# uniio/ivf-hnsw

Hardware: AMD Instinct MI355X
Metric: queries/sec @ Recall@1, SIFT1B PQ16 nprobe=32; ADC scan HBM GB/s vs peak (higher is better)
Workload: dtype f32

## Files before the change

### ivf-hnsw_amd/csrc/capi_internal.h

```cpp
#pragma once
#include "../../include/ivfhnsw_hip.h"
#include "ivfhnsw_kernels.h"

#include <hip/hip_runtime.h>

#include <algorithm>
#include <new>
#include <cmath>
#include <cstddef>
#include <cstdio>
#include <cstdlib>
#include <cstring>
#include <functional>
#include <string>
#include <unordered_map>
#include <vector>

namespace ivfhnsw_gpu_impl {

int fail(int code, const char *fmt, ...) __attribute__((format(printf, 2, 3)));

#define HIP_TRY(expr)                                                                                        \
    do {                                                                                                     \
        hipError_t e_ = (expr);                                                                              \
// ... 359 lines not shown
        if (!on)
            return;
        (void)hipEventRecord(ev.b, s);
        h->pending.push_back(ev);
    }
};

constexpr uint32_t kHeapStreamCap = 8192;

constexpr int kSplitAuto = 1000;

constexpr size_t kMaxBatchAll = 1 << 17;

struct EarlyTables {
    hipStream_t stream;
    hipEvent_t ready;
    hipEvent_t done;
};

struct SearchCall {
    uint32_t *status_out = nullptr;
    bool defer_redo = false;
    bool no_latency = false;
    bool wrote_status = false;
    const EarlyTables *early = nullptr;
};

struct WalkClear {
    uint64_t *keys = nullptr;
    uint32_t *done = nullptr;
    bool cleared = false;
};

struct SearchArgs {
    size_t nq, k;
    const float *d_queries;
    const uint32_t *d_coarse_ids;
    const float *d_coarse_dists;
    const ivfhnsw_search_params *p;
    float *d_distances;
    int64_t *d_labels, *d_out_keys;
    const uint8_t *d_query_slots = nullptr;
    SearchArgs slice(size_t q0, size_t n, size_t d) const
    {
        return {n, k, d_queries + q0 * d, d_coarse_ids ? d_coarse_ids + q0 * p->nprobe : nullptr,
                d_coarse_dists ? d_coarse_dists + q0 * p->nprobe : nullptr, p, d_distances + q0 * k, d_labels + q0 * k,
                d_out_keys, d_query_slots ? d_query_slots + q0 : nullptr};
    }
};

struct Chunk : SearchArgs {
    int nprobe, max_seg, plan_k;
    bool heap_big;
    ScanFilter fmask;
    const float *xq;
    const uint32_t *cid;
    const float *cd;
    bool use_tail;
    WalkClear meet;
    int nsplit;
    bool heap, pipe;
    const EarlyTables *early;
};

int search_args_guard(const ivfhnsw_gpu *h, const ivfhnsw_search_params *p, size_t k);
int stage_in(ivfhnsw_gpu *h, DevBuf &b, const void *src, size_t bytes);
int stage_out(ivfhnsw_gpu *h, void *dst, const DevBuf &b, size_t bytes);
int chunk_checks(ivfhnsw_gpu *h, const Chunk &c, bool results = true);
int chunk_workspace(ivfhnsw_gpu *h, Chunk &c);
int chunk_coarse(ivfhnsw_gpu *h, Chunk &c, const SearchCall &call);
int chunk_plan_table(ivfhnsw_gpu *h, Chunk &c);

void base_filter_drop(ivfhnsw_gpu *h);
int base_filter_cols(ivfhnsw_gpu *h, const ivfhnsw_gpu *b, SweepCols *cols, size_t *nx);

void base_slots_drop(ivfhnsw_gpu *h);
int base_slots_table_write(ivfhnsw_gpu *h, bool create);
int base_slots_call(ivfhnsw_gpu *h, const ivfhnsw_gpu *b, const char *who, const StripCols **table, unsigned *forms);

void range_drop(ivfhnsw_gpu *h);

int grouping_dedupe_reserve(ivfhnsw_gpu *h);
int grouping_dedupe_dev(ivfhnsw_gpu *h, const uint32_t *d_sizes, const uint32_t *d_nn, int *dedupe);

int encode_rows(ivfhnsw_gpu *h, size_t m, float *dx, const float *table, const uint32_t *rows);
int encode_groups_impl(ivfhnsw_gpu *h, size_t ngroups, size_t nsubc, const uint32_t *centroid_idx,
                       const uint64_t *offsets, const float *x, size_t efSearch, uint32_t *out_nn_centroid_idxs,
                       float *out_alphas, uint32_t *out_subcentroid_idxs, uint8_t *out_codes, uint8_t *out_norm_codes,
                       bool dev, bool stage);

}
```

### ivf-hnsw_amd/csrc/capi_search.cpp

```cpp
#include "capi_internal.h"

static size_t env_size(const char *name, size_t def)
{
    const char *e = getenv(name);
    return (e && *e) ? (size_t)atol(e) : def;
}

int ivfhnsw_gpu_impl::search_args_guard(const ivfhnsw_gpu *h, const ivfhnsw_search_params *p, size_t k)
{
    if (!h->has_ivf)
        return fail(IVFHNSW_ERR_STATE, "search before upload_ivf");
    if (!p || p->nprobe == 0 || k == 0)
        return fail(IVFHNSW_ERR_INVALID, "nprobe and k must be positive");
    return IVFHNSW_OK;
}

int ivfhnsw_gpu_impl::stage_in(ivfhnsw_gpu *h, DevBuf &b, const void *src, size_t bytes)
{
    int rc = b.ensure(bytes);
    if (rc)
        return rc;
    HIP_TRY(hipMemcpyAsync(b.p, src, bytes, hipMemcpyHostToDevice, h->stream));
    return IVFHNSW_OK;
}

int ivfhnsw_gpu_impl::stage_out(ivfhnsw_gpu *h, void *dst, const DevBuf &b, size_t bytes)
{
    HIP_TRY(hipMemcpyAsync(dst, b.p, bytes, hipMemcpyDeviceToHost, h->stream));
    return IVFHNSW_OK;
}

static int walk_scratch(ivfhnsw_gpu *h, size_t words, size_t nslots, size_t nq, uint32_t **tails)
{
    int rc = h->w_visited.ensure(words * sizeof(uint32_t) * std::max<size_t>(nslots, 64) * 2);
    if (rc)
        return rc;
    if (h->w_visited.p != h->walk.zero_ptr || h->w_visited.bytes != h->walk.zero_bytes) {
        HIP_TRY(hipMemsetAsync(h->w_visited.p, 0, h->w_visited.bytes, h->stream));
        h->walk.zero = true;
        h->walk.zero_ptr = h->w_visited.p;
        h->walk.zero_bytes = h->w_visited.bytes;
    }
    *tails = reinterpret_cast<uint32_t *>(h->w_visited.as<char>() + h->w_visited.bytes / 2);
    return h->w_redo.ensure(nq * sizeof(uint32_t));
}

static int coarse_dev_impl(ivfhnsw_gpu *h, size_t nq, const float *d_queries, size_t nprobe, size_t efSearch,
                           uint32_t *d_coarse_ids, float *d_coarse_dists, const SearchCall &call, WalkClear &meet)
{
    int rc = bind(h);
    if (rc)
        return rc;
    if (!h->has_graph)
        return fail(IVFHNSW_ERR_STATE, "coarse search needs upload_quantizer");
    if (nprobe == 0 || efSearch < nprobe)
        return fail(IVFHNSW_ERR_INVALID, "efSearch %zu < nprobe %zu (precondition of IndexIVF_HNSW.cpp:249-258)",
                    efSearch, nprobe);
    if (efSearch > 1024)
        return fail(IVFHNSW_ERR_INVALID, "efSearch %zu > 1024 unsupported on the device", efSearch);
    if (nq == 0)
        return IVFHNSW_OK;
    if (nq > 0x7fffffffull)
        return fail(IVFHNSW_ERR_INVALID, "nq too large");
    const size_t words = ((((size_t)h->gr.n + 31) / 32) + 3) & ~(size_t)3;
    StageScope sc(h, IVFHNSW_STAGE_COARSE);
    static const size_t lat_max_nq = env_size("IVFHNSW_LATENCY_MAX_NQ", 256);
    StatusWords *st = status_words(h);
    uint32_t *tails = nullptr;
    if (!call.no_latency && nq <= lat_max_nq && coarse_latency_supported(h->gr, (int)efSearch)) {
        uint32_t *hdr = &st->redo_len;
        const bool defer = call.defer_redo;
        if (!defer) {
            if ((rc = walk_scratch(h, words, 64, nq, &tails)))
                return rc;
            HIP_TRY(hipMemsetAsync(hdr, 0, 3 * sizeof(uint32_t), h->stream));
        }
        HIP_TRY(launch_coarse_latency(h->stream, h->gr, d_queries, (int)nq, (int)nprobe, (int)efSearch, d_coarse_ids,
                                      d_coarse_dists, status_word(h), meet.keys, meet.done, defer ? nullptr : hdr,
                                      defer ? nullptr : h->w_redo.as<uint32_t>()));
        meet.cleared = meet.keys != nullptr;
        if (!defer)
            HIP_TRY(launch_coarse_redo(h->stream, h->gr, d_queries, (int)nq, (int)nprobe, (int)efSearch, d_coarse_ids,
                                       d_coarse_dists, h->w_visited.as<uint32_t>(), words, status_word(h), hdr,
                                       h->w_redo.as<uint32_t>(), tails, 64));
        return IVFHNSW_OK;
    }
    const int nslots = (int)std::min<size_t>(nq, (size_t)coarse_slots_for((int)efSearch));
    if ((rc = walk_scratch(h, words, (size_t)nslots, nq, &tails)))
        return rc;
    HIP_TRY(launch_coarse(h->stream, h->gr, d_queries, (int)nq, (int)nprobe, (int)efSearch, d_coarse_ids, d_coarse_dists,
                          h->w_visited.as<uint32_t>(), words, nslots, status_word(h), &st->walk_next,
                          h->w_visited.bytes / 2, &h->walk.zero, h->w_redo.as<uint32_t>(), tails, 64,
                          &h->walk.counters_clean));
    return IVFHNSW_OK;
}

int ivfhnsw_gpu_coarse_dev(ivfhnsw_gpu *h, size_t nq, const float *d_queries, size_t nprobe, size_t efSearch,
                           uint32_t *d_coarse_ids, float *d_coarse_dists)
{
    WalkClear meet;
    return coarse_dev_impl(h, nq, d_queries, nprobe, efSearch, d_coarse_ids, d_coarse_dists, SearchCall(), meet);
}

int ivfhnsw_gpu_rotate_dev(ivfhnsw_gpu *h, size_t nq, const float *d_queries, float *d_out)
{
    int rc = bind(h);
    if (rc)
        return rc;
    if (!h->has_ivf)
        return fail(IVFHNSW_ERR_STATE, "rotate needs upload_ivf");
    if (nq == 0)
        return IVFHNSW_OK;
    if (!d_queries || !d_out || nq > 0x7fffffffull)
        return fail(IVFHNSW_ERR_INVALID, "null buffer or nq too large");
    if (h->t.opq_At) {
        StageScope sc(h, IVFHNSW_STAGE_OPQ);
        HIP_TRY(launch_opq(h->stream, h->t.opq_At, d_queries, d_out, (int)nq, h->t.d));
    } else if (d_out != d_queries) {
        HIP_TRY(hipMemcpyAsync(d_out, d_queries, nq * (size_t)h->t.d * sizeof(float), hipMemcpyDeviceToDevice, h->stream));
    }
    return IVFHNSW_OK;
}

int ivfhnsw_gpu_coarse(ivfhnsw_gpu *h, size_t nq, const float *queries, size_t k, size_t efSearch, uint32_t *ids,
                       float *dists)
{
// ... 225 lines not shown
    return IVFHNSW_OK;
}

int ivfhnsw_gpu_impl::chunk_coarse(ivfhnsw_gpu *h, Chunk &c, const SearchCall &call)
{
    const size_t nq = c.nq;
    int rc;
    c.xq = c.d_queries;
    if (h->t.opq_At) {
        if ((rc = h->w_xq.ensure(nq * (size_t)h->t.d * sizeof(float))))
            return rc;
        {
            StageScope sc(h, IVFHNSW_STAGE_OPQ);
            HIP_TRY(launch_opq(h->stream, h->t.opq_At, c.d_queries, h->w_xq.as<float>(), (int)nq, h->t.d));
        }
        c.xq = h->w_xq.as<float>();
        if (call.early) {
            HIP_TRY(hipEventRecord(call.early->ready, h->stream));
            HIP_TRY(hipStreamWaitEvent(call.early->stream, call.early->ready, 0));
        }
    }
    static const size_t tail_max_nq = env_size("IVFHNSW_TAIL_MAX_NQ", 8);
    c.use_tail = !h->has_group && nq <= tail_max_nq && !c.d_out_keys && !c.fmask.any() &&
                 ivf_tail_supported(h->t, c.nprobe, (int)c.k);
    if (c.use_tail) {
        if ((rc = h->w_tail.ensure(nq * (sizeof(uint64_t) + sizeof(uint32_t)))))
            return rc;
        c.meet.keys = h->w_tail.as<uint64_t>();
        c.meet.done = reinterpret_cast<uint32_t *>(c.meet.keys + nq);
    }
    c.cid = c.d_coarse_ids;
    c.cd = c.d_coarse_dists;
    if (!c.cid) {
        if ((rc = h->w_cid.ensure(nq * (size_t)c.nprobe * sizeof(uint32_t))) ||
            (rc = h->w_cd.ensure(nq * (size_t)c.nprobe * sizeof(float))) ||
            (rc = coarse_dev_impl(h, nq, c.xq, c.p->nprobe, c.p->efSearch, h->w_cid.as<uint32_t>(), h->w_cd.as<float>(),
                                  call, c.meet)))
            return rc;
        c.cid = h->w_cid.as<uint32_t>();
        c.cd = h->w_cd.as<float>();
    }
    return IVFHNSW_OK;
}

static int chunk_tail(ivfhnsw_gpu *h, const Chunk &c, SearchCall &call)
{
    const size_t nq = c.nq;
    const int nsplit = (int)std::min<size_t>(32, (2048 + nq - 1) / nq);
    StageScope sc(h, IVFHNSW_STAGE_SCAN);
    if (!c.meet.cleared)
        HIP_TRY(hipMemsetAsync(c.meet.keys, 0, nq * (sizeof(uint64_t) + sizeof(uint32_t)), h->stream));
    HIP_TRY(launch_ivf_tail(h->stream, h->t, c.xq, c.cid, c.cd, (int)nq, c.nprobe, c.p->max_codes, nsplit, c.meet.keys,
                            c.meet.done, h->w_hdr.as<PlanHdr>(), c.d_distances, c.d_labels, status_word(h),
                            call.status_out));
    call.wrote_status = call.status_out != nullptr;
    remember_plan(h, nq, c.max_seg, false, "ivf_tail_kernel");
    return IVFHNSW_OK;
}

int ivfhnsw_gpu_impl::chunk_plan_table(ivfhnsw_gpu *h, Chunk &c)
{
    const int nq = (int)c.nq, max_seg = c.max_seg;
    const ivfhnsw_search_params *p = c.p;
    int rc;
    c.heap = p->heap_order && c.k > 1;
    c.nsplit = (c.k == 1 && c.nq < 1024) ? (int)std::min<size_t>(32, (2048 + c.nq - 1) / c.nq) : 1;
    c.pipe = c.k == 1 && !h->has_group && !c.heap && !c.fmask.any() && h->opt_scan_pipe != 0 &&
             scan_pipe_supported(h->t, max_seg, nq, c.nsplit, h->n_local > 0, h->opt_scan_pipe == 1);
    const bool plan_lut = !c.pipe && plan_lut_shape(h);
    if (!c.pipe && (rc = h->w_luts.ensure(c.nq * (size_t)h->t.M * 256 * sizeof(float))))
        return rc;
    const PlanView plan = plan_of(h, max_seg, c.nq);
    uint64_t *keys = h->w_keys.as<uint64_t>();
    if (plan_lut && c.early) {
        const EarlyTables &e = *c.early;
        {
            StageScope sc(h, IVFHNSW_STAGE_LUT, e.stream);
            HIP_TRY(launch_lut(e.stream, h->t, c.xq, h->w_luts.as<float>(), nq, nullptr));
        }
        HIP_TRY(hipEventRecord(e.done, e.stream));
        {
            StageScope sc(h, IVFHNSW_STAGE_PLAN);
            HIP_TRY(launch_plan_ivf(h->stream, h->t, c.cid, c.cd, c.nprobe, p->max_codes, plan, keys, c.plan_k));
        }
        HIP_TRY(hipStreamWaitEvent(h->stream, e.done, 0));
        return IVFHNSW_OK;
    }
    if (plan_lut) {
        StageScope sc(h, IVFHNSW_STAGE_LUT);
        HIP_TRY(launch_plan_lut(h->stream, h->t, c.xq, c.cid, c.cd, c.nprobe, p->max_codes, plan, keys, c.plan_k,
                                h->w_luts.as<float>()));
        return IVFHNSW_OK;
    }
    {
        StageScope sc(h, IVFHNSW_STAGE_PLAN);
        if (h->has_group) {
            if ((rc = h->w_qsd.ensure(c.nq * (size_t)max_seg * 2 * sizeof(float))))
                return rc;
            HIP_TRY(launch_plan_grouping(h->stream, h->t, h->g, h->gr, c.xq, c.cid, c.cd, c.nprobe, p->max_codes,
                                         p->do_pruning, plan, keys, c.plan_k, h->w_qsd.as<float>()));
        } else {
            HIP_TRY(launch_plan_ivf(h->stream, h->t, c.cid, c.cd, c.nprobe, p->max_codes, plan, keys, c.plan_k));
        }
    }
    if (!c.pipe) {
        StageScope sc(h, IVFHNSW_STAGE_LUT);
        HIP_TRY(launch_lut(h->stream, h->t, c.xq, h->w_luts.as<float>(), nq, plan.hdr));
    }
    return IVFHNSW_OK;
}

static int chunk_scan_select(ivfhnsw_gpu *h, const Chunk &c)
{
    const int k = (int)c.k;
    const bool heap = c.heap, replay_here = c.heap && !c.d_out_keys;
    float *luts = h->w_luts.as<float>();
    const PlanView plan = plan_of(h, c.max_seg, c.nq);
    int rc;
    float *heap_ws = nullptr;
    if (replay_here) {
        if ((rc = h->w_heap.ensure(heap_scan_ws_bytes(h->t.M, k, plan.nq))))
            return rc;
        heap_ws = h->w_heap.as<float>();
    }
    if (c.heap_big) {
        {
            StageScope sc(h, IVFHNSW_STAGE_SCAN);
            HIP_TRY(launch_heap_scan(h->stream, h->t, luts, plan, k, nullptr, nullptr, heap_ws, c.d_distances, c.d_labels,
                                     c.fmask));
        }
        remember_plan(h, c.nq, c.max_seg, false, c.fmask.name("heap_scan_kernel", "heap_scan_kernel+filter", "heap_scan_kernel+slots"));
        return IVFHNSW_OK;
    }
    if (heap) {
        if ((rc = h->w_stream.ensure(c.nq * (size_t)kHeapStreamCap * sizeof(uint64_t))) ||
// ... 263 lines not shown
```

### ivf-hnsw_amd/csrc/ivfhnsw_kernels.h

```cpp
#pragma once

#include <hip/hip_runtime.h>
#include <mutex>
#include <stdint.h>

#include "scan_dispatch.h"
#include "sweep_plan_math.h"
#include "update_math.h"

namespace ivfhnsw_gpu_impl {

struct DynLdsState {
    std::mutex m;
    size_t raised[64] = {};
};
inline hipError_t raise_dyn_lds(const void *kern, size_t bytes, DynLdsState &st)
{
    int dev = 0;
    hipError_t e = hipGetDevice(&dev);
    if (e != hipSuccess)
        return e;
    if (dev < 0 || dev >= 64)
        return hipFuncSetAttribute(kern, hipFuncAttributeMaxDynamicSharedMemorySize, (int)bytes);
    std::lock_guard<std::mutex> lk(st.m);
// ... 123 lines not shown
                       const char **kernel_name);
bool scan_pipe_supported(const IvfTables &t, int max_seg, int nq, int nsplit, bool has_codes, bool forced = false);
hipError_t launch_scan_pipe(hipStream_t s, const IvfTables &t, const float *xq, const PlanView &p, uint64_t *keys);
bool ivf_tail_supported(const IvfTables &t, int nprobe, int k);
hipError_t launch_ivf_tail(hipStream_t s, const IvfTables &t, const float *xq, const uint32_t *cid, const float *cd,
                           int nq, int nprobe, uint64_t max_codes, int nsplit, uint64_t *keys_inv, uint32_t *done,
                           PlanHdr *hdr, float *dist, int64_t *labels, const uint32_t *status_word, uint32_t *status_out);
hipError_t launch_heap_replay(hipStream_t s, const IvfTables &t, const PlanView &p, const uint64_t *stream,
                              const uint32_t *stream_len, uint32_t stream_cap, int k, float *dist, int64_t *labels,
                              uint32_t *status,
                              int64_t *out_keys = nullptr,
                              uint32_t *redo_hdr = nullptr, uint32_t *redo_list = nullptr);
bool heap_scan_lds_tier(int code_size, int k);
size_t heap_scan_ws_bytes(int code_size, int k, int nq);
hipError_t launch_heap_scan(hipStream_t s, const IvfTables &t, const float *luts, const PlanView &p, int k,
                            uint32_t *redo_hdr, const uint32_t *redo_list, float *heap_ws, float *dist, int64_t *labels,
                            const ScanFilter &fmask = ScanFilter());
hipError_t launch_range_count(hipStream_t s, const IvfTables &t, const float *luts, const PlanView &p, int nsplit,
                              int seg_len_hint, float radius, uint32_t *slices, unsigned long long *total,
                              const ScanFilter &fmask, const char **kernel_name);
hipError_t launch_range_lims(hipStream_t s, const uint32_t *bases, int nq, int nsplit, uint64_t *lims);
hipError_t launch_range_fill(hipStream_t s, const IvfTables &t, const float *luts, const PlanView &p, int nsplit,
                             int seg_len_hint, float radius, const uint32_t *bases, float *dist, int64_t *labels,
                             const ScanFilter &fmask);
hipError_t launch_select(hipStream_t s, const IvfTables &t, const PlanView &p, const uint64_t *keys, int k, float *dist,
                         int64_t *labels, int64_t *out_keys);
hipError_t launch_resolve(hipStream_t s, const IvfTables &t, const PlanView &p, const int64_t *skeys, int k, float *dist,
                          int64_t *labels);
hipError_t launch_coarse(hipStream_t s, const GraphTables &g, const float *xq, int nq, int nprobe, int ef,
                         uint32_t *coarse_ids, float *coarse_dists, uint32_t *visited_scratch,
                         size_t visited_words_per_slot, int nslots, uint32_t *status, uint32_t *next_query,
                         size_t visited_bytes = 0, bool *visited_zero = nullptr,
                         uint32_t *redo_list = nullptr, uint32_t *tail_bitmaps = nullptr, int tail_slots = 0,
                         bool *counters_clean = nullptr);
hipError_t launch_coarse_redo(hipStream_t s, const GraphTables &g, const float *xq, int nq, int nprobe, int ef,
                              uint32_t *coarse_ids, float *coarse_dists, uint32_t *visited_scratch,
                              size_t visited_words_per_slot, uint32_t *status, uint32_t *redo_hdr, uint32_t *redo_list,
                              uint32_t *tail_bitmaps, int tail_slots);
int coarse_slots_for(int ef);
bool coarse_latency_supported(const GraphTables &g, int ef);
size_t coarse_latency_fat_bytes(const GraphTables &g);
hipError_t launch_build_fat(hipStream_t s, const GraphTables &g, float *fat);
hipError_t launch_coarse_latency(hipStream_t s, const GraphTables &g, const float *xq, int nq, int nprobe, int ef,
                                 uint32_t *coarse_ids, float *coarse_dists, uint32_t *status,
                                 uint64_t *zero_keys = nullptr, uint32_t *zero_done = nullptr,
                                 uint32_t *redo_hdr = nullptr, uint32_t *redo_list = nullptr);
constexpr uint32_t kStatusHnswTieOverflow = 1u;
constexpr uint32_t kStatusTopkStreamOverflow = 2u;
hipError_t launch_madd_rows(hipStream_t s, const float *a, float bf, const float *table, const uint32_t *idx, float *c,
                            size_t n, int d);
hipError_t launch_pq_encode(hipStream_t s, const float *r, const float *cb, uint8_t *codes, size_t n, int d, int M);
hipError_t launch_pq_decode(hipStream_t s, const uint8_t *codes, const float *cb, float *dec, size_t n, int d, int M);
hipError_t launch_norm_codes(hipStream_t s, const float *rec, const float *ntab, uint8_t *norm_codes, float *norms_out,
                             size_t n, int d);
constexpr int kXtyChunk = 2048;
hipError_t launch_lloyd_update(hipStream_t s, const float *x, const uint8_t *assign, float *cb, size_t n, int d, int M);
hipError_t launch_xty(hipStream_t s, const float *X, const float *Y, float *partials, float *C, size_t n, int d);
constexpr int kKmeansTile = 4096;
hipError_t launch_kmeans_count(hipStream_t s, const uint32_t *assign, const float *dist, size_t n, uint32_t nc,
                               uint32_t *cnt, double *part, uint32_t *status);
hipError_t launch_scan_u32(hipStream_t s, const uint32_t *in, uint32_t *out, size_t len);
hipError_t launch_sort_by_key(hipStream_t s, const uint32_t *keys, size_t n, int key_bits, uint32_t *ids_a, uint32_t *ids_b,
                              uint32_t *hist, uint32_t **sorted);
hipError_t launch_sort_by_key_from(hipStream_t s, const uint32_t *keys, size_t n, int key_bits, const uint32_t *start,
                                   uint32_t *ids_a, uint32_t *ids_b, uint32_t *hist, uint32_t **sorted);
hipError_t launch_kmeans_means(hipStream_t s, const float *x, size_t n, const uint32_t *members, const uint32_t *start,
                               const uint32_t *cnt, float *c, size_t nc, int d);
hipError_t launch_kmeans_split(hipStream_t s, float *c, const uint32_t *pairs, size_t npairs, int d);
inline int knn_splits_for(size_t nq, size_t nx) { return sweep_splits_for(nq, nx, 128); }
hipError_t launch_knn_norms(hipStream_t s, const float *x, float *out, size_t n, int d);
hipError_t launch_knn(hipStream_t s, const float *Q, const float *X, const float *qn, const float *xn, size_t nq, size_t nx,
// ... 116 lines not shown
```

### ivf-hnsw_amd/csrc/kernels_hnsw.hip

```cpp
#include "ivfhnsw_kernels.h"
#include "device_common.h"
#include "walk_set.h"

#include <float.h>
#include <stdio.h>
#include <stdlib.h>

namespace ivfhnsw_gpu_impl {

constexpr int vis_buckets(int minw, int tagw = 8)
{
    return minw <= 4 ? (tagw == 10 ? 1040 : 1008) : minw == 5 ? 768 : minw <= 7 ? 640 : 384;
}

template <int TAGW> struct VisFields {
    static constexpr int cntw = TAGW == 8 ? 8 : TAGW == 10 ? 14 : 16;
    static constexpr int cshift = 64 - cntw;
    static constexpr int slots = cshift / TAGW;
    static constexpr unsigned long long ones()
    {
        unsigned long long o = 0;
        for (int i = 0; i < slots; i++)
            o |= 1ull << (TAGW * i);
        return o;
    }
};

template <int TAGW, int NB>
__device__ __forceinline__ bool visit_test_and_set(uint32_t id, unsigned long long *vt, uint32_t *bm, bool &used_bitmap)
{
    if constexpr (TAGW != 0) {
        using F = VisFields<TAGW>;
        constexpr unsigned long long kOnes = F::ones();
        constexpr unsigned long long kHighs = kOnes << (TAGW - 1);
// ... 70 lines not shown
        __builtin_amdgcn_sched_barrier(0);
#pragma unroll
        for (int i = 0; i < 4; i++) {
            if (j0 + 2 * i < nchunk) {
                const float4 *qq = reinterpret_cast<const float4 *>(sqp + 16 * (j0 + 2 * i));
                const uint32_t ws[4] = {w[i].x, w[i].y, w[i].z, w[i].w};
#pragma unroll
                for (int c = 0; c < 4; c++) {
                    const float4 qv = qq[c];
                    const float t0 = qv.x - (float)(ws[c] & 0xffu);
                    const float t1 = qv.y - (float)((ws[c] >> 8) & 0xffu);
                    const float t2 = qv.z - (float)((ws[c] >> 16) & 0xffu);
                    const float t3 = qv.w - (float)(ws[c] >> 24);
                    a0 = fmaf(t0, t0, a0);
                    a1 = fmaf(t1, t1, a1);
                    a2 = fmaf(t2, t2, a2);
                    a3 = fmaf(t3, t3, a3);
                }
            }
        }
    }
    return (a0 + a1) + (a2 + a3);
}

__device__ __forceinline__ unsigned long long walk_stamp()
{
    __builtin_amdgcn_sched_barrier(0);
    const unsigned long long t = __builtin_amdgcn_s_memtime();
    __builtin_amdgcn_s_waitcnt(0xC07F);
    __builtin_amdgcn_sched_barrier(0);
    return t;
}

template <int NCH, int MINW, int TAGW, int FMODE, bool STAMPS = false, bool SPILL = false>
__global__ __launch_bounds__(64, MINW) void hnsw_walk_kernel(GraphTables g, const float *__restrict__ xq, int nq, int nprobe,
                                                       int ef, uint32_t *__restrict__ coarse_ids,
                                                       float *__restrict__ coarse_dists,
                                                       uint32_t *__restrict__ visited, size_t vwords,
                                                       uint32_t *__restrict__ status, uint32_t *__restrict__ next_query,
                                                       uint32_t *__restrict__ redo_hdr, uint32_t *__restrict__ redo_list,
                                                       uint32_t *__restrict__ tail_bitmaps = nullptr,
                                                       unsigned long long *__restrict__ stamp_out = nullptr)
{
    extern __shared__ __attribute__((aligned(16))) unsigned char smem[];
    float *s_q = reinterpret_cast<float *>(smem);
    float *s_qp = s_q + g.d;
    const int dp = FMODE == 1 ? g.d : 0;
    uint32_t *s_q8 = reinterpret_cast<uint32_t *>(s_qp + dp);
    unsigned long long *tail = reinterpret_cast<unsigned long long *>(smem + (size_t)(g.d + dp) * sizeof(float) + 512);
    constexpr int NB = vis_buckets(MINW, TAGW);
    unsigned long long st_acc[9] = {0, 0, 0, 0, 0, 0}, st_t = 0;
    const int merge_extra = (NCH <= 4 && ef + 8 > kTailCap) ? ef + 8 - kTailCap : 0;
    unsigned long long *vt = tail + kTailCap + merge_extra;
    constexpr bool LDSVIS = TAGW != 0;

    const int lane = threadIdx.x;
    const int judged_row = 8 * (((lane >> 2) & 1) * 2 + (lane & 1)) + (lane >> 3);
    const bool merge_on = g.merge_admissions != 0;
    constexpr bool prefilter = FMODE != 0;
    constexpr bool inline_rows = FMODE >= 2;
    constexpr bool ROWNORMS = FMODE == 3;
    constexpr bool CK = FMODE >= 2;
    auto enc_id = [](uint32_t id, uint32_t c) { return CK ? (id << 7) | c : id; };
    auto dec_id = [](uint32_t e) { return CK ? e >> 7 : e; };
    uint32_t *bm = visited + (size_t)blockIdx.x * vwords;
    TailSpill spill;
    spill.bm = SPILL ? tail_bitmaps + (size_t)blockIdx.x * vwords : nullptr;
    spill.hi = -1;
    spill.count = 0;
    bool bitmap_dirty = !(LDSVIS && g.visited_clean);
    bool redo_ran = false;

    for (;;) {
        int q = 0;
        if constexpr (SPILL) {
            if (lane == 0) {
                const uint32_t i = atomicAdd(&redo_hdr[1], 1u);
                q = i < redo_hdr[0] ? (int)redo_list[i] : nq;
            }
        } else {
            if (lane == 0)
                q = (int)atomicAdd(next_query, 1u);
        }
        q = __builtin_amdgcn_readfirstlane(q);
        if (q >= nq)
            break;
        redo_ran = true;
        if (STAMPS)
            st_t = walk_stamp();

        if (!LDSVIS || bitmap_dirty) {
            uint4 *bm4 = reinterpret_cast<uint4 *>(bm);
            const size_t v4 = vwords / 4;
            for (size_t w = lane; w < v4; w += 64)
                bm4[w] = make_uint4(0u, 0u, 0u, 0u);
            bitmap_dirty = false;
        }
        if (LDSVIS)
            for (int w = lane; w < NB; w += 64)
                vt[w] = 0ull;
        __syncthreads();
        float qp_sq = 0.f;
        for (int i = lane; i < g.d; i += 64) {
            const float v = xq[(size_t)q * g.d + i];
            s_q[i] = v;
            if (prefilter) {
                const float vp = __fdiv_rn(__fsub_rn(v, g.q_lo), g.q_step);
// ... 472 lines not shown
                        } else {
                            if (lane == 0)
                                redo_list[atomicAdd(&redo_hdr[0], 1u)] = (uint32_t)q;
                            ntail = -1;
                            break;
                        }
                    }
                }
                if (STAMPS) {
                    const unsigned long long t = walk_stamp();
                    st_acc[3] += t - st_t;
                    st_t = t;
                }
            }
            if (ntail < 0)
                break;
        }

        if (SPILL && spill.count > 0)
            spill.clear(lane);
        if (LDSVIS && __ballot(used_bitmap))
            bitmap_dirty = true;
        if (ntail >= 0) {
#pragma unroll
            for (int cc = 0; cc < NCH; cc++) {
                const int i = cc * 64 + lane;
                if (i < nprobe) {
                    const bool have = i < n;
                    coarse_ids[(size_t)q * nprobe + i] = have ? dec_id(key_id(R.r[cc])) : 0xffffffffu;
                    coarse_dists[(size_t)q * nprobe + i] = have ? __uint_as_float(key_dist_bits(R.r[cc])) : 0.f;
                }
            }
        }
    }
    if constexpr (SPILL) {
        if (lane == 0) {
            __threadfence();
            if (atomicAdd(&redo_hdr[2], 1u) == gridDim.x - 1) {
                redo_hdr[-1] = 0;
                redo_hdr[0] = 0;
                redo_hdr[1] = 0;
                redo_hdr[2] = 0;
            }
        }
    }
    if (SPILL && redo_ran) {
        uint4 *bm4 = reinterpret_cast<uint4 *>(bm);
        for (size_t w = lane; w < vwords / 4; w += 64)
            bm4[w] = make_uint4(0u, 0u, 0u, 0u);
    }
    if (LDSVIS && bitmap_dirty) {
        uint4 *bm4 = reinterpret_cast<uint4 *>(bm);
        for (size_t w = lane; w < vwords / 4; w += 64)
            bm4[w] = make_uint4(0u, 0u, 0u, 0u);
    }
    if (STAMPS && stamp_out && lane == 0)
        for (int i = 0; i < 9; i++)
            atomicAdd(&stamp_out[i], st_acc[i]);
}

__global__ __launch_bounds__(64) void build_nbrows_kernel(GraphTables g, uint8_t *__restrict__ nbrows,
                                                          uint32_t *__restrict__ nbnorms, int nb_rows,
                                                          uint32_t *__restrict__ links_c)
{
    const size_t node = blockIdx.x;
    const int cnt = g.counts[node];
    if ((int)threadIdx.x < g.maxM) {
        uint32_t e = 0;
// ... 11 lines not shown
            v = reinterpret_cast<const uint4 *>(g.qrows + (size_t)g.links[node * g.maxM + r] * g.d)[c];
        reinterpret_cast<uint4 *>(nbrows + (node * nb_rows + r) * 128)[c] = v;
        uint32_t rr = 0;
        rr = __builtin_amdgcn_udot4(v.x, v.x, rr, false);
        rr = __builtin_amdgcn_udot4(v.y, v.y, rr, false);
        rr = __builtin_amdgcn_udot4(v.z, v.z, rr, false);
        rr = __builtin_amdgcn_udot4(v.w, v.w, rr, false);
        rr = (uint32_t)oct_sum((int)rr);
        if (c == 0)
            nbnorms[node * nb_rows + r] = rr;
    }
}

hipError_t launch_build_nbrows(hipStream_t s, const GraphTables &g, uint8_t *nbrows, uint32_t *nbnorms, int nb_rows,
                               uint32_t *links_c)
{
    if (!g.qrows || g.d > 128 || (g.d & 15) || nb_rows < g.maxM || (nb_rows & 31) || g.n >= (1u << 24) || g.maxM > 64)
        return hipErrorInvalidValue;
    hipLaunchKernelGGL(build_nbrows_kernel, dim3(g.n), dim3(64), 0, s, g, nbrows, nbnorms, nb_rows, links_c);
    return hipGetLastError();
}

int coarse_slots_for(int ef)
{
    const int nch = (ef + 63) / 64;
    const int waves_per_simd = nch <= 8 ? 4 : 3;
    return 256 * 4 * waves_per_simd;
}

hipError_t launch_coarse(hipStream_t s, const GraphTables &g_in, const float *xq, int nq, int nprobe, int ef,
                         uint32_t *coarse_ids, float *coarse_dists, uint32_t *visited_scratch,
                         size_t visited_words_per_slot, int nslots, uint32_t *status, uint32_t *next_query,
                         size_t visited_bytes, bool *visited_zero, uint32_t *redo_list, uint32_t *tail_bitmaps,
                         int tail_slots, bool *counters_clean)
{
    if (nq == 0)
        return hipSuccess;
    GraphTables g = g_in;
    if (ef > 1024 || ef < 1 || nprobe > ef || g.maxM > 64 || g.n >= 0x80000000u || (visited_words_per_slot & 3) ||
        !redo_list || !tail_bitmaps || tail_slots < 1)
        return hipErrorInvalidValue;
    uint32_t *redo_hdr = next_query + 1;
    hipError_t e = hipSuccess;
    if (!counters_clean || !*counters_clean) {
        e = hipMemsetAsync(next_query, 0, 4 * sizeof(uint32_t), s);
        if (e != hipSuccess)
            return e;
    }
    if (counters_clean)
        *counters_clean = false;
    constexpr int occ = 4;
    const int nch = (ef + 63) / 64;
    const int occ_eff = 4;
    uint32_t nbk = (uint32_t)vis_buckets(occ_eff);
    static const bool force_bitmap = [] {
        const char *e = getenv("IVFHNSW_WALK_VIS");
        return e && e[0] == 'b';
    }();
    int tagw = force_bitmap ? 0 : g.n <= 255u * nbk ? 8 : g.n <= 4095u * nbk ? 12 : g.n <= 65535u * nbk ? 16 : 0;
    static const int force_tagw = [] {
        const char *e = getenv("IVFHNSW_WALK_TAGW");
        const int v = e ? atoi(e) : 0;
        return (v == 10 || v == 12 || v == 16) ? v : 0;
    }();
    if (tagw && force_tagw > tagw)
        tagw = force_tagw;
    if ((tagw == 12 || tagw == 10) && occ_eff == 4 && g.n <= 1023u * (uint32_t)vis_buckets(4, 10) && force_tagw != 12) {
// ... 67 lines not shown
                    fprintf(stderr, "[walk stamps] rows evaluated/expansion %.2f, passing the wave-wide test %.2f, admitted %.2f\n",
                            (double)h[6] / h[5], (double)h[7] / h[5], (double)h[8] / h[5]);
                }
            });
        }
        if (tagw == 8)
            hipLaunchKernelGGL((hnsw_walk_kernel<2, 4, 8, 2, true>), dim3(nslots), dim3(64), shm, s, g, xq, nq, nprobe, ef,
                               coarse_ids, coarse_dists, visited_scratch, visited_words_per_slot, status, next_query, redo_hdr,
                               redo_list, nullptr, d_st);
        else
            hipLaunchKernelGGL((hnsw_walk_kernel<2, 4, 10, 3, true>), dim3(nslots), dim3(64), shm, s, g, xq, nq, nprobe, ef,
                               coarse_ids, coarse_dists, visited_scratch, visited_words_per_slot, status, next_query, redo_hdr,
                               redo_list, nullptr, d_st);
        return hipGetLastError();
    }
    if (nch <= 1) {
        IVFHNSW_WALK_N(1);
    } else if (nch <= 2) {
        IVFHNSW_WALK_N(2);
    } else if (nch == 3) {
        IVFHNSW_WALK_N(3);
    } else if (nch <= 4) {
        IVFHNSW_WALK_N(4);
    } else if (nch <= 8) {
        IVFHNSW_WALK(8, 4);
    } else {
        IVFHNSW_WALK(16, 4);
    }
#undef IVFHNSW_WALK_N
#undef IVFHNSW_WALK
#undef IVFHNSW_WALK_T
#undef IVFHNSW_WALK_F
    e = hipGetLastError();
    if (e != hipSuccess)
        return e;
    e = launch_coarse_redo(s, g, xq, nq, nprobe, ef, coarse_ids, coarse_dists, visited_scratch, visited_words_per_slot,
                           status, redo_hdr, redo_list, tail_bitmaps, tail_slots);
    if (e == hipSuccess && counters_clean)
        *counters_clean = true;
    return e;
}

hipError_t launch_coarse_redo(hipStream_t s, const GraphTables &g_in, const float *xq, int nq, int nprobe, int ef,
                              uint32_t *coarse_ids, float *coarse_dists, uint32_t *visited_scratch,
                              size_t visited_words_per_slot, uint32_t *status, uint32_t *redo_hdr, uint32_t *redo_list,
                              uint32_t *tail_bitmaps, int tail_slots)
{
    GraphTables g = g_in;
    g.visited_clean = 0;
    const int nch = (ef + 63) / 64;
    const int slots = std::min(std::min(nq, tail_slots), 64);
    const size_t shm = (size_t)g.d * sizeof(float) + 512 +
                       (size_t)(kTailCap + ((ef <= 256 && ef + 8 > kTailCap) ? ef + 8 - kTailCap : 0)) * sizeof(unsigned long long);
#define IVFHNSW_REDO(N)                                                                                               \
    hipLaunchKernelGGL((hnsw_walk_kernel<N, 4, 0, 0, false, true>), dim3(slots), dim3(64), shm, s, g, xq, nq, nprobe, ef, \
                       coarse_ids, coarse_dists, visited_scratch, visited_words_per_slot, status, redo_hdr + 1, redo_hdr, \
                       redo_list, tail_bitmaps)
    if (nch <= 1)
        IVFHNSW_REDO(1);
    else if (nch <= 2)
        IVFHNSW_REDO(2);
    else if (nch == 3)
        IVFHNSW_REDO(3);
    else if (nch <= 4)
        IVFHNSW_REDO(4);
    else if (nch <= 8)
        IVFHNSW_REDO(8);
    else
        IVFHNSW_REDO(16);
#undef IVFHNSW_REDO
    return hipGetLastError();
}

}
```

### ivf-hnsw_amd/csrc/kernels_search.hip

```cpp
#include "plan_steps.h"
#include "scan_steps.h"
#include "sweep_steps.h"

#include <float.h>
#include <stdlib.h>
#include <algorithm>

namespace ivfhnsw_gpu_impl {

__global__ void opq_kernel(const float *__restrict__ At, const float *__restrict__ x, float *__restrict__ y, int nq,
                           int d)
{
    extern __shared__ float s_x[];
    const int q = blockIdx.x;
    for (int i = threadIdx.x; i < d; i += blockDim.x)
        s_x[i] = x[(size_t)q * d + i];
    __syncthreads();
    for (int i = threadIdx.x; i < d; i += blockDim.x) {
        float acc = 0.0f;
        for (int k = 0; k < d; k++)
            acc = __fmaf_rn(At[(size_t)k * d + i], s_x[k], acc);
        y[(size_t)q * d + i] = acc;
    }
}
// ... 100 lines not shown
    lut_body<DSUB>((int)blockIdx.x, s_q, xq, cb, luts, nq, d, M, dsub_rt, hdr);
}

hipError_t launch_lut(hipStream_t s, const IvfTables &t, const float *xq, float *luts, int nq, const PlanHdr *hdr)
{
    if (nq == 0)
        return hipSuccess;
    dim3 grid((nq + LUT_QB - 1) / LUT_QB), block(256);
    size_t shm = (size_t)LUT_QB * t.d * sizeof(float);
    switch (t.dsub) {
    case 4: hipLaunchKernelGGL(lut_kernel<4>, grid, block, shm, s, xq, t.pq_centroids, luts, nq, t.d, t.M, t.dsub, hdr); break;
    case 6: hipLaunchKernelGGL(lut_kernel<6>, grid, block, shm, s, xq, t.pq_centroids, luts, nq, t.d, t.M, t.dsub, hdr); break;
    case 8: hipLaunchKernelGGL(lut_kernel<8>, grid, block, shm, s, xq, t.pq_centroids, luts, nq, t.d, t.M, t.dsub, hdr); break;
    case 12: hipLaunchKernelGGL(lut_kernel<12>, grid, block, shm, s, xq, t.pq_centroids, luts, nq, t.d, t.M, t.dsub, hdr); break;
    case 16: hipLaunchKernelGGL(lut_kernel<16>, grid, block, shm, s, xq, t.pq_centroids, luts, nq, t.d, t.M, t.dsub, hdr); break;
    default:
        if (t.dsub > 64)
            return hipErrorInvalidValue;
        hipLaunchKernelGGL(lut_kernel<0>, grid, block, shm, s, xq, t.pq_centroids, luts, nq, t.d, t.M, t.dsub, hdr);
    }
    return hipGetLastError();
}

__device__ __forceinline__ void plan_ivf_body(int bid, const IvfTables &t, const uint32_t *__restrict__ cid,
                                              const float *__restrict__ cd, int nq, int nprobe,
                                              unsigned long long max_codes, Seg *__restrict__ segs,
                                              uint32_t *__restrict__ lpos, PlanHdr *__restrict__ hdr, int max_seg,
                                              unsigned long long *__restrict__ keys, int k)
{
    const int q = bid * 4 + (threadIdx.x >> 6);
    const int lane = threadIdx.x & 63;
    if (q >= nq)
        return;
    for (int j = lane; j < k; j += 64)
        keys[(size_t)q * k + j] = kKeyInit;
    PlanCursor cur;
    for (int base = 0; base < nprobe && plan_budget_open(cur.ncode, max_codes); base += 64)
        ivf_plan_chunk(cur, t, cid + (size_t)q * nprobe, cd + (size_t)q * nprobe, base, nprobe, max_codes,
                       segs + (size_t)q * max_seg, lpos + (size_t)q * max_seg, lane);
    if (lane == 0)
        store_plan_hdr(&hdr[q], cur.ns, cur.nl);
}

__global__ __launch_bounds__(256) void plan_ivf_kernel(IvfTables t, const uint32_t *__restrict__ cid,
                                                       const float *__restrict__ cd, int nq, int nprobe,
                                                       unsigned long long max_codes, Seg *__restrict__ segs,
                                                       uint32_t *__restrict__ lpos, PlanHdr *__restrict__ hdr,
                                                       int max_seg, unsigned long long *__restrict__ keys, int k)
{
    plan_ivf_body((int)blockIdx.x, t, cid, cd, nq, nprobe, max_codes, segs, lpos, hdr, max_seg, keys, k);
}

template <int DSUB>
__global__ __launch_bounds__(256) void plan_lut_kernel(IvfTables t, const uint32_t *__restrict__ cid,
                                                       const float *__restrict__ cd, int nq, int nprobe,
                                                       unsigned long long max_codes, Seg *__restrict__ segs,
                                                       uint32_t *__restrict__ lpos, PlanHdr *__restrict__ hdr,
                                                       int max_seg, unsigned long long *__restrict__ keys, int k,
                                                       int plan_blocks, const float *__restrict__ xq,
                                                       float *__restrict__ luts)
{
    extern __shared__ float s_q[];
    if ((int)blockIdx.x < plan_blocks)
        plan_ivf_body((int)blockIdx.x, t, cid, cd, nq, nprobe, max_codes, segs, lpos, hdr, max_seg, keys, k);
    else
        lut_body<DSUB>((int)blockIdx.x - plan_blocks, s_q, xq, t.pq_centroids, luts, nq, t.d, t.M, t.dsub, nullptr);
}

hipError_t launch_plan_lut(hipStream_t s, const IvfTables &t, const float *xq, const uint32_t *coarse_ids,
                           const float *coarse_dists, int nprobe, uint64_t max_codes, const PlanView &p, uint64_t *keys,
                           int k, float *luts)
{
    const auto [segs, lpos, hdr, max_seg, nq] = p;
    if (nq == 0)
// ... 525 lines not shown
```

### ivf-hnsw_amd/csrc/plan_steps.h

```cpp
#pragma once

#include "ivfhnsw_kernels.h"
#include "device_common.h"
#include "plan_math.h"

namespace ivfhnsw_gpu_impl {

struct PlanCursor {
    unsigned long long ncode = 0;
    uint32_t ns = 0, nl = 0;
};

__device__ __forceinline__ void store_plan_hdr(PlanHdr *dst, uint32_t ns, uint32_t nl)
{
    PlanHdr h;
    h.nseg = ns;
    h.total = nl;
    *dst = h;
}

__device__ __forceinline__ float ivf_cterm(float coarse_dist, float centroid_norm)
{
    return __fsub_rn(coarse_dist, centroid_norm);
}
// ... 2 lines not shown
                                               const float *__restrict__ qd, int base, int nprobe,
                                               unsigned long long max_codes, Seg *sq, uint32_t *lq, int lane)
{
    const int i = base + lane;
    uint32_t c = 0xffffffffu;
    if (i < nprobe)
        c = qc[i];
    const bool ok = c < t.nc;
    unsigned long long n = 0;
    if (ok)
        n = t.goff[c + 1] - t.goff[c];
    const unsigned long long incl = wave_incl_scan_u64(n, lane) + cur.ncode;
    const unsigned long long excl = incl - n;
    const bool take = plan_takes_list(n, excl, max_codes);
    const uint32_t lo_c = take ? t.loff[c] : kNotOwned;
    const bool owned = lo_c != kNotOwned;
    const unsigned long long om = __ballot(owned);
    const unsigned long long own_incl = wave_incl_scan_u64(owned ? n : 0ull, lane);
    if (owned) {
        const uint32_t r = cur.ns + (uint32_t)__popcll(om & ((1ull << lane) - 1ull));
        Seg sg;
        sg.start = lo_c;
        sg.len = (uint32_t)n;
        sg.vpos = (uint32_t)excl;
        sg.cterm = ivf_cterm(qd[i], t.centroid_norms[c]);
        sq[r] = sg;
        lq[r] = cur.nl + (uint32_t)(own_incl - n);
    }
    cur.ns += (uint32_t)__popcll(om);
    cur.nl += (uint32_t)__shfl(own_incl, 63, 64);
    const unsigned long long stop = __ballot(take && plan_pass2_ends(incl, max_codes));
    const int last = stop ? __ffsll((long long)stop) - 1 : 63;
    cur.ncode = __shfl(incl, last, 64);
}

struct GroupTerms {
    float alpha, oma, term1;
};
__device__ __forceinline__ GroupTerms group_terms(float alpha, float x)
{
    const float oma = __fsub_rn(1.0f, alpha);
    return GroupTerms{alpha, oma, __fmul_rn(oma, x)};
}
__device__ __forceinline__ float group_pass1_value(const GroupTerms &gt, float inter, float qn)
{
    const float a = __fmul_rn(gt.oma, inter);
    const float b = __fsub_rn(a, qn);
    return __fsub_rn(gt.term1, __fmul_rn(gt.alpha, b));
}
__device__ __forceinline__ float group_cterm(const GroupTerms &gt, float qn, float nn_norm)
{
    const float term2 = __fmul_rn(gt.alpha, __fsub_rn(qn, nn_norm));
    return __fadd_rn(gt.term1, term2);
}

__device__ __forceinline__ void wave_lds_order()
{
    asm volatile("s_waitcnt lgkmcnt(0)" ::: "memory");
}

template <bool FOUR_WAVES>
__device__ __forceinline__ float gather_quads(bool ask, unsigned long long am, uint32_t nn, float held,
                                              const float *__restrict__ vectors, const float *s_q, int d, float *s_dist,
                                              int lane)
{
    const int na = __popcll(am);
// ... 79 lines not shown
```

Baseline: 6.188 million.

## Fuse coarse redo pass with IVF plan construction into one walk kernel

Defers the coarse HNSW redo launch and runs it inside a new plan kernel. Each block builds the IVF plan for its own query if that query is not on the redo list. The first 64 blocks then work through redo queries via the walk kernel and plan each one right after re-walking it. This removes a separate kernel launch and a dependency gap between coarse redo and planning. The cost is a larger, more register-heavy walk kernel that launches one block per query, which may hurt occupancy and adds cross-block counter-reset logic.

```diff
diff --git a/ivf-hnsw_amd/csrc/capi_internal.h b/ivf-hnsw_amd/csrc/capi_internal.h
--- a/ivf-hnsw_amd/csrc/capi_internal.h
+++ b/ivf-hnsw_amd/csrc/capi_internal.h
@@ -415,6 +415,12 @@
     bool cleared = false;
 };
 
+struct RedoLater {
+    bool want = false, pending = false;
+    size_t words = 0;
+    uint32_t *tails = nullptr;
+};
+
 struct SearchArgs {
     size_t nq, k;
     const float *d_queries;
@@ -441,6 +447,7 @@
     const float *cd;
     bool use_tail;
     WalkClear meet;
+    RedoLater redo;
     int nsplit;
     bool heap, pipe;
     const EarlyTables *early;
diff --git a/ivf-hnsw_amd/csrc/capi_search.cpp b/ivf-hnsw_amd/csrc/capi_search.cpp
--- a/ivf-hnsw_amd/csrc/capi_search.cpp
+++ b/ivf-hnsw_amd/csrc/capi_search.cpp
@@ -46,7 +46,8 @@
 }
 
 static int coarse_dev_impl(ivfhnsw_gpu *h, size_t nq, const float *d_queries, size_t nprobe, size_t efSearch,
-                           uint32_t *d_coarse_ids, float *d_coarse_dists, const SearchCall &call, WalkClear &meet)
+                           uint32_t *d_coarse_ids, float *d_coarse_dists, const SearchCall &call, WalkClear &meet,
+                           RedoLater *later = nullptr)
 {
     int rc = bind(h);
     if (rc)
@@ -88,10 +89,16 @@
     const int nslots = (int)std::min<size_t>(nq, (size_t)coarse_slots_for((int)efSearch));
     if ((rc = walk_scratch(h, words, (size_t)nslots, nq, &tails)))
         return rc;
+    const bool redo_later = later && later->want;
     HIP_TRY(launch_coarse(h->stream, h->gr, d_queries, (int)nq, (int)nprobe, (int)efSearch, d_coarse_ids, d_coarse_dists,
                           h->w_visited.as<uint32_t>(), words, nslots, status_word(h), &st->walk_next,
                           h->w_visited.bytes / 2, &h->walk.zero, h->w_redo.as<uint32_t>(), tails, 64,
-                          &h->walk.counters_clean));
+                          &h->walk.counters_clean, redo_later));
+    if (redo_later) {
+        later->pending = true;
+        later->words = words;
+        later->tails = tails;
+    }
     return IVFHNSW_OK;
 }
 
@@ -383,10 +390,12 @@
     c.cid = c.d_coarse_ids;
     c.cd = c.d_coarse_dists;
     if (!c.cid) {
+        static const bool redo_in_plan = env_size("IVFHNSW_REDO_IN_PLAN", 1) != 0;
+        c.redo.want = redo_in_plan && !c.use_tail && !h->has_group && h->t.shard_world == 1 && !c.d_out_keys;
         if ((rc = h->w_cid.ensure(nq * (size_t)c.nprobe * sizeof(uint32_t))) ||
             (rc = h->w_cd.ensure(nq * (size_t)c.nprobe * sizeof(float))) ||
             (rc = coarse_dev_impl(h, nq, c.xq, c.p->nprobe, c.p->efSearch, h->w_cid.as<uint32_t>(), h->w_cd.as<float>(),
-                                  call, c.meet)))
+                                  call, c.meet, &c.redo)))
             return rc;
         c.cid = h->w_cid.as<uint32_t>();
         c.cd = h->w_cd.as<float>();
@@ -423,6 +432,26 @@
         return rc;
     const PlanView plan = plan_of(h, max_seg, c.nq);
     uint64_t *keys = h->w_keys.as<uint64_t>();
+    uint32_t *redo_hdr = &status_words(h)->redo_len;
+    auto plan_ivf = [&]() -> int {
+        if (!c.redo.pending) {
+            HIP_TRY(launch_plan_ivf(h->stream, h->t, c.cid, c.cd, c.nprobe, p->max_codes, plan, keys, c.plan_k));
+            return IVFHNSW_OK;
+        }
+        HIP_TRY(launch_plan_redo(h->stream, h->t, h->gr, c.xq, c.nprobe, (int)p->efSearch, h->w_cid.as<uint32_t>(),
+                                 h->w_cd.as<float>(), h->w_visited.as<uint32_t>(), c.redo.words, status_word(h), redo_hdr,
+                                 h->w_redo.as<uint32_t>(), c.redo.tails, 64, p->max_codes, plan, keys, c.plan_k));
+        c.redo.pending = false;
+        h->walk.counters_clean = true;
+        return IVFHNSW_OK;
+    };
+    if (c.redo.pending && !(plan_lut && c.early) && (plan_lut || h->has_group)) {
+        HIP_TRY(launch_coarse_redo(h->stream, h->gr, c.xq, nq, c.nprobe, (int)p->efSearch, h->w_cid.as<uint32_t>(),
+                                   h->w_cd.as<float>(), h->w_visited.as<uint32_t>(), c.redo.words, status_word(h), redo_hdr,
+                                   h->w_redo.as<uint32_t>(), c.redo.tails, 64));
+        c.redo.pending = false;
+        h->walk.counters_clean = true;
+    }
     if (plan_lut && c.early) {
         const EarlyTables &e = *c.early;
         {
@@ -432,7 +461,8 @@
         HIP_TRY(hipEventRecord(e.done, e.stream));
         {
             StageScope sc(h, IVFHNSW_STAGE_PLAN);
-            HIP_TRY(launch_plan_ivf(h->stream, h->t, c.cid, c.cd, c.nprobe, p->max_codes, plan, keys, c.plan_k));
+            if ((rc = plan_ivf()))
+                return rc;
         }
         HIP_TRY(hipStreamWaitEvent(h->stream, e.done, 0));
         return IVFHNSW_OK;
@@ -450,8 +480,8 @@
                 return rc;
             HIP_TRY(launch_plan_grouping(h->stream, h->t, h->g, h->gr, c.xq, c.cid, c.cd, c.nprobe, p->max_codes,
                                          p->do_pruning, plan, keys, c.plan_k, h->w_qsd.as<float>()));
-        } else {
-            HIP_TRY(launch_plan_ivf(h->stream, h->t, c.cid, c.cd, c.nprobe, p->max_codes, plan, keys, c.plan_k));
+        } else if ((rc = plan_ivf())) {
+            return rc;
         }
     }
     if (!c.pipe) {
diff --git a/ivf-hnsw_amd/csrc/ivfhnsw_kernels.h b/ivf-hnsw_amd/csrc/ivfhnsw_kernels.h
--- a/ivf-hnsw_amd/csrc/ivfhnsw_kernels.h
+++ b/ivf-hnsw_amd/csrc/ivfhnsw_kernels.h
@@ -179,11 +179,17 @@
                          size_t visited_words_per_slot, int nslots, uint32_t *status, uint32_t *next_query,
                          size_t visited_bytes = 0, bool *visited_zero = nullptr,
                          uint32_t *redo_list = nullptr, uint32_t *tail_bitmaps = nullptr, int tail_slots = 0,
-                         bool *counters_clean = nullptr);
+                         bool *counters_clean = nullptr,
+                         bool redo_later = false);
 hipError_t launch_coarse_redo(hipStream_t s, const GraphTables &g, const float *xq, int nq, int nprobe, int ef,
                               uint32_t *coarse_ids, float *coarse_dists, uint32_t *visited_scratch,
                               size_t visited_words_per_slot, uint32_t *status, uint32_t *redo_hdr, uint32_t *redo_list,
                               uint32_t *tail_bitmaps, int tail_slots);
+hipError_t launch_plan_redo(hipStream_t s, const IvfTables &t, const GraphTables &g, const float *xq, int nprobe, int ef,
+                            uint32_t *coarse_ids, float *coarse_dists, uint32_t *visited_scratch,
+                            size_t visited_words_per_slot, uint32_t *status, uint32_t *redo_hdr, uint32_t *redo_list,
+                            uint32_t *tail_bitmaps, int tail_slots, uint64_t max_codes, const PlanView &p, uint64_t *keys,
+                            int k);
 int coarse_slots_for(int ef);
 bool coarse_latency_supported(const GraphTables &g, int ef);
 size_t coarse_latency_fat_bytes(const GraphTables &g);
diff --git a/ivf-hnsw_amd/csrc/kernels_hnsw.hip b/ivf-hnsw_amd/csrc/kernels_hnsw.hip
--- a/ivf-hnsw_amd/csrc/kernels_hnsw.hip
+++ b/ivf-hnsw_amd/csrc/kernels_hnsw.hip
@@ -1,5 +1,6 @@
 #include "ivfhnsw_kernels.h"
 #include "device_common.h"
+#include "plan_steps.h"
 #include "walk_set.h"
 
 #include <float.h>
@@ -136,7 +137,15 @@
     return t;
 }
 
-template <int NCH, int MINW, int TAGW, int FMODE, bool STAMPS = false, bool SPILL = false>
+struct PlanInWalk {
+    IvfTables t;
+    unsigned long long max_codes;
+    PlanView p;
+    unsigned long long *keys;
+    int k;
+};
+
+template <int NCH, int MINW, int TAGW, int FMODE, bool STAMPS = false, bool SPILL = false, class... Plan>
 __global__ __launch_bounds__(64, MINW) void hnsw_walk_kernel(GraphTables g, const float *__restrict__ xq, int nq, int nprobe,
                                                        int ef, uint32_t *__restrict__ coarse_ids,
                                                        float *__restrict__ coarse_dists,
@@ -144,8 +153,27 @@
                                                        uint32_t *__restrict__ status, uint32_t *__restrict__ next_query,
                                                        uint32_t *__restrict__ redo_hdr, uint32_t *__restrict__ redo_list,
                                                        uint32_t *__restrict__ tail_bitmaps = nullptr,
-                                                       unsigned long long *__restrict__ stamp_out = nullptr)
-{
+                                                       unsigned long long *__restrict__ stamp_out = nullptr, Plan... plan)
+{
+    constexpr bool IN_PLAN = sizeof...(Plan) != 0;
+    static_assert(!IN_PLAN || (SPILL && sizeof...(Plan) == 1), "the plan launch carries the redo form");
+    [[maybe_unused]] bool lends = true;
+    if constexpr (IN_PLAN) {
+        const PlanInWalk &pl = (plan, ...);
+        const int own = blockIdx.x;
+        const uint32_t nlisted = redo_hdr[0];
+        if (own == 0 && threadIdx.x == 0)
+            *next_query = 0;
+        bool listed = false;
+        for (uint32_t i = threadIdx.x; i < nlisted; i += 64)
+            listed |= redo_list[i] == (uint32_t)own;
+        if (!__any(listed))
+            plan_ivf_query(own, (int)threadIdx.x, pl.t, coarse_ids, coarse_dists, nprobe, pl.max_codes, pl.p.segs, pl.p.lpos,
+                           pl.p.hdr, pl.p.max_seg, pl.keys, pl.k);
+        if (nlisted == 0)
+            return;
+        lends = blockIdx.x < 64u;
+    }
     extern __shared__ __attribute__((aligned(16))) unsigned char smem[];
     float *s_q = reinterpret_cast<float *>(smem);
     float *s_qp = s_q + g.d;
@@ -177,6 +205,9 @@
 
     for (;;) {
         int q = 0;
+        if constexpr (IN_PLAN)
+            if (!lends)
+                break;
         if constexpr (SPILL) {
             if (lane == 0) {
                 const uint32_t i = atomicAdd(&redo_hdr[1], 1u);
@@ -715,8 +746,23 @@
                 }
             }
         }
-    }
-    if constexpr (SPILL) {
+        if constexpr (IN_PLAN) {
+            const PlanInWalk &pl = (plan, ...);
+            __threadfence();
+            plan_ivf_query(q, lane, pl.t, coarse_ids, coarse_dists, nprobe, pl.max_codes, pl.p.segs, pl.p.lpos, pl.p.hdr,
+                           pl.p.max_seg, pl.keys, pl.k);
+        }
+    }
+    if constexpr (IN_PLAN) {
+        if (lane == 0) {
+            __threadfence();
+            if (atomicAdd(&redo_hdr[2], 1u) == gridDim.x - 1) {
+                redo_hdr[0] = 0;
+                redo_hdr[1] = 0;
+                redo_hdr[2] = 0;
+            }
+        }
+    } else if constexpr (SPILL) {
         if (lane == 0) {
             __threadfence();
             if (atomicAdd(&redo_hdr[2], 1u) == gridDim.x - 1) {
@@ -794,7 +840,7 @@
                          uint32_t *coarse_ids, float *coarse_dists, uint32_t *visited_scratch,
                          size_t visited_words_per_slot, int nslots, uint32_t *status, uint32_t *next_query,
                          size_t visited_bytes, bool *visited_zero, uint32_t *redo_list, uint32_t *tail_bitmaps,
-                         int tail_slots, bool *counters_clean)
+                         int tail_slots, bool *counters_clean, bool redo_later)
 {
     if (nq == 0)
         return hipSuccess;
@@ -928,7 +974,7 @@
 #undef IVFHNSW_WALK_T
 #undef IVFHNSW_WALK_F
     e = hipGetLastError();
-    if (e != hipSuccess)
+    if (e != hipSuccess || redo_later)
         return e;
     e = launch_coarse_redo(s, g, xq, nq, nprobe, ef, coarse_ids, coarse_dists, visited_scratch, visited_words_per_slot,
                            status, redo_hdr, redo_list, tail_bitmaps, tail_slots);
@@ -968,4 +1014,41 @@
     return hipGetLastError();
 }
 
-}
+hipError_t launch_plan_redo(hipStream_t s, const IvfTables &t, const GraphTables &g_in, const float *xq, int nprobe, int ef,
+                            uint32_t *coarse_ids, float *coarse_dists, uint32_t *visited_scratch,
+                            size_t visited_words_per_slot, uint32_t *status, uint32_t *redo_hdr, uint32_t *redo_list,
+                            uint32_t *tail_bitmaps, int tail_slots, uint64_t max_codes, const PlanView &p, uint64_t *keys,
+                            int k)
+{
+    if (p.nq == 0)
+        return hipSuccess;
+    if (tail_slots < 64 || !redo_list || !tail_bitmaps)
+        return hipErrorInvalidValue;
+    GraphTables g = g_in;
+    g.visited_clean = 0;
+    const int nch = (ef + 63) / 64;
+    const size_t shm = (size_t)g.d * sizeof(float) + 512 +
+                       (size_t)(kTailCap + ((ef <= 256 && ef + 8 > kTailCap) ? ef + 8 - kTailCap : 0)) * sizeof(unsigned long long);
+    const PlanInWalk pl{t, (unsigned long long)max_codes, p, reinterpret_cast<unsigned long long *>(keys), k};
+    unsigned long long *no_stamps = nullptr;
+#define IVFHNSW_PLAN_REDO(N)                                                                                          \
+    hipLaunchKernelGGL((hnsw_walk_kernel<N, 4, 0, 0, false, true, PlanInWalk>), dim3(p.nq), dim3(64), shm, s, g, xq,  \
+                       p.nq, nprobe, ef, coarse_ids, coarse_dists, visited_scratch, visited_words_per_slot, status,   \
+                       redo_hdr - 1, redo_hdr, redo_list, tail_bitmaps, no_stamps, pl)
+    if (nch <= 1)
+        IVFHNSW_PLAN_REDO(1);
+    else if (nch <= 2)
+        IVFHNSW_PLAN_REDO(2);
+    else if (nch == 3)
+        IVFHNSW_PLAN_REDO(3);
+    else if (nch <= 4)
+        IVFHNSW_PLAN_REDO(4);
+    else if (nch <= 8)
+        IVFHNSW_PLAN_REDO(8);
+    else
+        IVFHNSW_PLAN_REDO(16);
+#undef IVFHNSW_PLAN_REDO
+    return hipGetLastError();
+}
+
+}
diff --git a/ivf-hnsw_amd/csrc/kernels_search.hip b/ivf-hnsw_amd/csrc/kernels_search.hip
--- a/ivf-hnsw_amd/csrc/kernels_search.hip
+++ b/ivf-hnsw_amd/csrc/kernels_search.hip
@@ -156,14 +156,7 @@
     const int lane = threadIdx.x & 63;
     if (q >= nq)
         return;
-    for (int j = lane; j < k; j += 64)
-        keys[(size_t)q * k + j] = kKeyInit;
-    PlanCursor cur;
-    for (int base = 0; base < nprobe && plan_budget_open(cur.ncode, max_codes); base += 64)
-        ivf_plan_chunk(cur, t, cid + (size_t)q * nprobe, cd + (size_t)q * nprobe, base, nprobe, max_codes,
-                       segs + (size_t)q * max_seg, lpos + (size_t)q * max_seg, lane);
-    if (lane == 0)
-        store_plan_hdr(&hdr[q], cur.ns, cur.nl);
+    plan_ivf_query(q, lane, t, cid, cd, nprobe, max_codes, segs, lpos, hdr, max_seg, keys, k);
 }
 
 __global__ __launch_bounds__(256) void plan_ivf_kernel(IvfTables t, const uint32_t *__restrict__ cid,
diff --git a/ivf-hnsw_amd/csrc/plan_steps.h b/ivf-hnsw_amd/csrc/plan_steps.h
--- a/ivf-hnsw_amd/csrc/plan_steps.h
+++ b/ivf-hnsw_amd/csrc/plan_steps.h
@@ -58,6 +58,22 @@
     const unsigned long long stop = __ballot(take && plan_pass2_ends(incl, max_codes));
     const int last = stop ? __ffsll((long long)stop) - 1 : 63;
     cur.ncode = __shfl(incl, last, 64);
+}
+
+__device__ __forceinline__ void plan_ivf_query(int q, int lane, const IvfTables &t, const uint32_t *__restrict__ cid,
+                                               const float *__restrict__ cd, int nprobe, unsigned long long max_codes,
+                                               Seg *__restrict__ segs, uint32_t *__restrict__ lpos,
+                                               PlanHdr *__restrict__ hdr, int max_seg,
+                                               unsigned long long *__restrict__ keys, int k)
+{
+    for (int j = lane; j < k; j += 64)
+        keys[(size_t)q * k + j] = kKeyInit;
+    PlanCursor cur;
+    for (int base = 0; base < nprobe && plan_budget_open(cur.ncode, max_codes); base += 64)
+        ivf_plan_chunk(cur, t, cid + (size_t)q * nprobe, cd + (size_t)q * nprobe, base, nprobe, max_codes,
+                       segs + (size_t)q * max_seg, lpos + (size_t)q * max_seg, lane);
+    if (lane == 0)
+        store_plan_hdr(&hdr[q], cur.ns, cur.nl);
 }
 
 struct GroupTerms {
```

After: 6.209 million (median of 6 runs). No clear change (+0.3%).
